# tjysdsg/speech-recognition

Hardware: AMD Instinct MI355X
Metric: frame-state loglik/s + utterances/s Viterbi decode (higher is better)
Workload: dtype f64; 1 GPU; configs[1]: 10-digit HMM, 5 states/digit, 8-mix GMM, 39-dim, 10000 utterances/GPU (999364 frames on rank 0), isolated-word decode; states=50, mixtures=8, dim=39, parallelism=utterance-sharded x1, batches_in_flight=2, process_group=single

## Files before the change

### speech-recognition_amd/csrc/gh_internal.h

```cpp
#pragma once
#include <hip/hip_runtime.h>
#include <stdint.h>
#include <stdarg.h>
#include <stdio.h>
#include <string>
#include <vector>
#include "../../include/gmmhmm.h"

void gh_set_error(const char* fmt, ...);

#define GH_HIP(call)                                                                     \
    do {                                                                                 \
        hipError_t e_ = (call);                                                          \
        if (e_ != hipSuccess) {                                                          \
            gh_set_error("%s:%d %s -> %s", __FILE__, __LINE__, #call, hipGetErrorString(e_)); \
            return (e_ == hipErrorOutOfMemory) ? GH_ERR_NOMEM : GH_ERR_HIP;              \
        }                                                                                \
    } while (0)

#define GH_REQUIRE(cond, ...)                 \
    do {                                      \
        if (!(cond)) {                        \
            gh_set_error(__VA_ARGS__);        \
            return GH_ERR_INVALID;            \
        }                                     \
    } while (0)

#define GH_LEAN_NARROW_ARCS 3

#define GH_LSE_SCALE64 184.66496523378731614
#define GH_LSE_SCALE32 1.4426950408889634074
#define GH_LSE_OFF64 (-1e300)
#define GH_LSE_OFF32 (-1e30f)
#define GH_LSE_COMPAT_BELOW64 (-745.1332191019412 * GH_LSE_SCALE64)
#define GH_LSE_BOUND_THR 0x1p-900
struct gh_lse_state { double k_mh, thr; };
__host__ __device__ inline gh_lse_state gh_lse_state_of(double mh, bool any_on, int M_pad) {
    gh_lse_state e;
    if (!any_on) { e.k_mh = 0.0; e.thr = INFINITY; return e; }
    e.k_mh = mh * GH_LSE_SCALE64;
    const double ex = (GH_LSE_COMPAT_BELOW64 - e.k_mh) * (1.0 / 128.0);
    const double t = (ex > 1000.0) ? (double)INFINITY : ((ex < -1060.0) ? 0.0 : ldexp(exp2(ex - floor(ex)), (int)floor(ex)) * (2.0 * M_pad));
    e.thr = (t > GH_LSE_BOUND_THR) ? t : GH_LSE_BOUND_THR;
    return e;
}
static inline int gh_lse_states_padded(int M_pad, int n_tiles) { return n_tiles * (16 / M_pad); }

struct gh_ctx {
    int device;
    hipStream_t stream;
    int n_cu;
    void* scratch;
    size_t scratch_bytes;
    int* d_flag;
    void* pinned;
    size_t pinned_bytes;
    double* d_fp64_tables;
    int compat;
    int last_fused = 0;
    int last_chunks;
    size_t budget_cache = 0;
    int budget_age = 0;
    void* fit_arena = nullptr;
    size_t fit_arena_bytes = 0;
    void* fit_pin = nullptr;
    void* fit_act = nullptr;
    size_t fit_act_bytes = 0;
};

int gh_scratch(gh_ctx* ctx, size_t bytes, void** out);
size_t gh_scratch_budget(gh_ctx* ctx, bool fresh = false);
int gh_pinned(gh_ctx* ctx, size_t bytes, void** out);

struct gh_gmm {
    gh_ctx* ctx;
    void* d_arena;
    int S, M, D, KP;
    std::vector<double> hA, hB, hC;
    bool host_stale = false;
    double *dA64, *dB64, *dC64;
    float *dA32, *dB32, *dC32;
    float* dCen32;
    double *dMean, *dIvar, *dLogc;
    int* dAnyPos = nullptr;
    int any_pos_host = -1;
    int M_pad, n_tiles;
    double *dApk64, *dCpk64;
    float *dApk32, *dCpk32;
    double* dCpkRel64 = nullptr;
    gh_lse_state* dLseState64 = nullptr;
    uint64_t serial = 0;
};
uint64_t gh_next_serial();

#define GH_FBCHAIN_MAX 16
struct gh_fbchain {
    int32_t n, pad;
    int32_t state[GH_FBCHAIN_MAX];
    double c0;
    double self_c[GH_FBCHAIN_MAX], next_c[GH_FBCHAIN_MAX], skip_c[GH_FBCHAIN_MAX];
};

struct gh_batch {
    gh_ctx* ctx;
    gh_dtype dtype;
    int D;
    int64_t N, U;
    void* feats;
    bool owns_feats;
    std::vector<int64_t> offsets;
    int64_t* d_offsets;
    int64_t max_T;
    bool any_T1 = false;
    void* nll;
    int nll_S;
    uint64_t nll_serial = 0;
    double* occ;
    int occ_S;
    int32_t* d_occ_states;
    double* gam;
    int gam_lanes = 0;
    bool occ_valid;
    std::vector<gh_fbchain> gam_chains;
    std::vector<int32_t> gam_utt_graph;
    std::vector<int64_t> perm;
    int64_t* d_perm;
    bool seq_seg_valid = false;
    std::vector<int32_t> seq_seg_lo, seq_seg_hi;
    std::vector<int32_t> seq_utt_K, seq_utt_word;
// ... 157 lines not shown
```

### speech-recognition_amd/csrc/gh_loglik_mfma.hip

```cpp
#include <type_traits>
#include "gh_internal.h"
#include "gh_wave.h"

namespace {

typedef double v4d __attribute__((ext_vector_type(4)));
typedef float v4f __attribute__((ext_vector_type(4)));

struct gh_loglik_blk { int64_t n0; int32_t nrows, t0, t1, pad; };

template <typename T> struct Acc;
template <> struct Acc<double> {
    typedef v4d type;
    static __device__ __forceinline__ v4d mfma(double a, double b, v4d c) {
        return __builtin_amdgcn_mfma_f64_16x16x4f64(a, b, c, 0, 0, 0);
    }
};
template <> struct Acc<float> {
    typedef v4f type;
    static __device__ __forceinline__ v4f mfma(float a, float b, v4f c) {
        return __builtin_amdgcn_mfma_f32_16x16x4f32(a, b, c, 0, 0, 0);
    }
};

struct Fp64Tables {
    double exp2[128];
    double inv[128];
    double nlog[128];
};

template <typename T> struct Dom;
template <> struct Dom<double> {
    static constexpr double inv_k = 1.0 / GH_LSE_SCALE64, off = GH_LSE_OFF64, off_test = GH_LSE_OFF64 * 0.1;
};
template <> struct Dom<float> {
    static constexpr float inv_k = (float)(1.0 / GH_LSE_SCALE32), off = GH_LSE_OFF32, off_test = GH_LSE_OFF32 * 0.1f;
};

struct LseK {
    double e3 = 2.6466421444330968834e-08;
    double l4 = -46.166241308446829036, l3 = 61.554988411262438714;
    double l2 = -92.332482616893658071, l1 = 184.66496523378731614;
    __device__ __forceinline__ void pin() {
        asm volatile("" : "+v"(e3), "+v"(l4), "+v"(l3), "+v"(l2), "+v"(l1));
    }
    __device__ __forceinline__ void pin_bnd() {
        asm volatile("" : "+v"(e3), "+v"(l4), "+s"(l3), "+s"(l2), "+s"(l1));
    }
};

__device__ __forceinline__ double logs(double s, const double* __restrict__ tab, const LseK& k) {
    const double* __restrict__ inv = tab + 128;
    const double* __restrict__ nlog = tab + 256;
    const double m = __builtin_amdgcn_frexp_mant(s);
    const int e = __builtin_amdgcn_frexp_exp(s);
    const int j = (__double2hiint(m) >> 13) & 127;
    const double rho = fma(m, inv[j], -1.0);
    double p = fma(rho, 36.932993046757463228, k.l4);
    p = fma(p, rho, k.l3);
    p = fma(p, rho, k.l2);
    p = fma(p, rho, k.l1);
    return fma(p, rho, nlog[j]) + (double)(e << 7);
}
__device__ __forceinline__ float logs(float s, const double*, const LseK&) { return __builtin_amdgcn_logf(s); }

template <int W> __device__ __forceinline__ void swap_rows(unsigned v, unsigned& a, unsigned& b) {
    if (W == 16) {
        auto r = __builtin_amdgcn_permlane16_swap(v, v, false, false);
        a = r[0]; b = r[1];
    } else {
        auto r = __builtin_amdgcn_permlane32_swap(v, v, false, false);
        a = r[0]; b = r[1];
    }
}
template <int W> __device__ __forceinline__ void pair_of(float v, float& a, float& b) {
    unsigned x, y;
    swap_rows<W>(__float_as_uint(v), x, y);
    a = __uint_as_float(x); b = __uint_as_float(y);
}
template <int W> __device__ __forceinline__ void pair_of(double v, double& a, double& b) {
    unsigned xl, yl, xh, yh;
    swap_rows<W>((unsigned)__double2loint(v), xl, yl);
    swap_rows<W>((unsigned)__double2hiint(v), xh, yh);
    a = __hiloint2double((int)xh, (int)xl); b = __hiloint2double((int)yh, (int)yl);
}
template <typename T, int W> __device__ __forceinline__ T pair_max(T v) { T a, b; pair_of<W>(v, a, b); return vmax(a, b); }
template <typename T, int W> __device__ __forceinline__ T pair_sum(T v) { T a, b; pair_of<W>(v, a, b); return a + b; }
__device__ __forceinline__ void pair_split(float v0, float v1, float& a, float& b) {
    auto r = __builtin_amdgcn_permlane16_swap(__float_as_uint(v0), __float_as_uint(v1), false, false);
    a = __uint_as_float(r[0]); b = __uint_as_float(r[1]);
}
__device__ __forceinline__ void pair_split(double v0, double v1, double& a, double& b) {
    auto lo = __builtin_amdgcn_permlane16_swap((unsigned)__double2loint(v0), (unsigned)__double2loint(v1), false, false);
    auto hi = __builtin_amdgcn_permlane16_swap((unsigned)__double2hiint(v0), (unsigned)__double2hiint(v1), false, false);
    a = __hiloint2double((int)hi[0], (int)lo[0]); b = __hiloint2double((int)hi[1], (int)lo[1]);
}
template <typename T> __device__ __forceinline__ T pair_sum_split(T v0, T v1) { T a, b; pair_split(v0, v1, a, b); return a + b; }
template <typename T> __device__ __forceinline__ T pair_max_split(T v0, T v1) { T a, b; pair_split(v0, v1, a, b); return vmax(a, b); }

template <typename T> __device__ __forceinline__ T nll_of(T mx, T sm, const double* tab, T inf_below, const LseK& k) {
    const T v = (mx + logs(sm, tab, k)) * -Dom<T>::inv_k;
    return (mx < inf_below) ? T(INFINITY) : v;
}

template <typename T, typename V> __device__ __forceinline__ T lane_max(const V& a) { return vmax(vmax(a[0], a[1]), vmax(a[2], a[3])); }
template <typename T, typename V> __device__ __forceinline__ T lane_terms(const V& a, T m, const double* tab, const LseK& k) {
    return (exp2s(a[0] - m, tab, k.e3) + exp2s(a[1] - m, tab, k.e3)) + (exp2s(a[2] - m, tab, k.e3) + exp2s(a[3] - m, tab, k.e3));
}
template <typename T, typename V>
__device__ __forceinline__ void tile_lse(const V& a, int width, T& mx, T& sm, const double* tab, const LseK& k) {
    T m = lane_max<T, V>(a);
    if (width >= 2) m = pair_max<T, 16>(m);
    if (width >= 4) m = pair_max<T, 32>(m);
    T e = lane_terms<T, V>(a, m, tab, k);
    if (width >= 2) e = pair_sum<T, 16>(e);
    if (width >= 4) e = pair_sum<T, 32>(e);
    mx = m;
    sm = e;
}

template <typename T, typename V, int W>
__device__ __forceinline__ void wide_lse(const V& acc0, const V& acc1, T& mxs, T& sm, const double* tab, const LseK& k) {
    mxs = pair_max_split(lane_max<T, V>(acc0), lane_max<T, V>(acc1));
    if (W >= 4) mxs = pair_max<T, 32>(mxs);
    T mx0, mx1;
    pair_of<16>(mxs, mx0, mx1);
    sm = pair_sum_split(lane_terms<T, V>(acc0, mx0, tab, k), lane_terms<T, V>(acc1, mx1, tab, k));
    if (W >= 4) sm = pair_sum<T, 32>(sm);
}

template <typename T, typename V> __device__ __forceinline__ T lane_terms0(const V& a, const double* tab, const LseK& k) {
    return (exp2s(a[0], tab, k.e3) + exp2s(a[1], tab, k.e3)) + (exp2s(a[2], tab, k.e3) + exp2s(a[3], tab, k.e3));
}
template <typename T> __device__ __forceinline__ T nll_bnd(T k_mh, T sm, const double* tab, const LseK& k) {
    return (k_mh + logs(sm, tab, k)) * -Dom<T>::inv_k;
}
template <typename T> __device__ __forceinline__ T nll_cold(T mx, T sm, T k_mh, const double* tab, T inf_below, const LseK& k) {
    const T v = ((mx + logs(sm, tab, k)) + k_mh) * -Dom<T>::inv_k;
    return (mx + k_mh < inf_below) ? T(INFINITY) : v;
}
__device__ __forceinline__ bool wave_any(bool p) { return __builtin_amdgcn_ballot_w64(p) != 0; }
__device__ __forceinline__ void cold_block() { asm volatile("; log-sum-exp redo (max-shifted)" ::: "memory"); }

__device__ __forceinline__ float exp2s_fe(double y) { return __builtin_amdgcn_exp2f((float)y * 0.0078125f); }
template <int W> __device__ __forceinline__ float pair_sum_f(float v) { float a, b; pair_of<W>(v, a, b); return a + b; }
// ... 136 lines not shown
            *((!CHK || s < S) ? orow0 + s : dummy) = nll_of_fe(mx, sm, inf_below);
            tile_lse_fe<V>(acc1, 1, mx, sm);
            *((!CHK || s < S) ? orow1 + s : dummy) = nll_of_fe(mx, sm, inf_below);
        }
    } else if (FE && MP <= 16) {
        if constexpr (FE) {
            constexpr int width = MP / 4;
            double mx0, mx1; float sm0, sm1;
            tile_lse_fe<V>(acc0, width, mx0, sm0);
            tile_lse_fe<V>(acc1, width, mx1, sm1);
            const bool odd = q & 1;
            const int s = (16 / MP) * t + q / width;
            const double v = nll_of_fe(odd ? mx1 : mx0, odd ? sm1 : sm0, inf_below);
            *(((q & (width - 1)) < 2 && (!CHK || s < S)) ? (odd ? orow1 : orow0) + s : dummy) = v;
        }
    } else if (FE) {
        if constexpr (FE) {
            const bool last = (t + 1) % tiles_per_state == 0;
            const int s = t / tiles_per_state;
#pragma unroll
            for (int c = 0; c < 2; ++c) {
                double mx; float smf;
                tile_lse_fe<V>(c ? acc1 : acc0, 4, mx, smf);
                const double d = run_mx[c] - mx;
                const float e = exp2s_fe((d > 0.0) ? -d : d);
                const float rs = (float)run_sm[c];
                run_sm[c] = (double)((d > 0.0) ? fmaf(smf, e, rs) : fmaf(rs, e, smf));
                run_mx[c] = (d > 0.0) ? run_mx[c] : mx;
            }
            const bool odd = q & 1;
            const double v = nll_of_fe(odd ? run_mx[1] : run_mx[0], (float)(odd ? run_sm[1] : run_sm[0]), inf_below);
            *((last && q < 2) ? (odd ? orow1 : orow0) + s : dummy) = v;
#pragma unroll
            for (int c = 0; c < 2; ++c) {
                run_mx[c] = last ? Dom<T>::off : run_mx[c];
                run_sm[c] = last ? T(0) : run_sm[c];
            }
        }
    } else if (MP == 4) {
        T mx, sm;
        const int s = 4 * t + q;
        tile_lse<T, V>(acc0, 1, mx, sm, tab, k);
        *((!CHK || s < S) ? orow0 + s : dummy) = nll_of<T>(mx, sm, tab, inf_below, k);
        tile_lse<T, V>(acc1, 1, mx, sm, tab, k);
        *((!CHK || s < S) ? orow1 + s : dummy) = nll_of<T>(mx, sm, tab, inf_below, k);
    } else if (MP <= 16) {
        constexpr int width = MP / 4;
        T mxs, sm;
        wide_lse<T, V, width>(acc0, acc1, mxs, sm, tab, k);
        const bool odd = q & 1;
        const int s = (16 / MP) * t + q / width;
        const T v = nll_of<T>(mxs, sm, tab, inf_below, k);
        *(((q & (width - 1)) < 2 && (!CHK || s < S)) ? (odd ? orow1 : orow0) + s : dummy) = v;
    } else {
        const bool last = (t + 1) % tiles_per_state == 0;
        const int s = t / tiles_per_state;
#pragma unroll
        for (int c = 0; c < 2; ++c) {
            T mx, sm;
            tile_lse<T, V>(c ? acc1 : acc0, 4, mx, sm, tab, k);
            const T d = run_mx[c] - mx;
            const T e = exp2s((d > T(0)) ? -d : d, tab, k.e3);
            run_sm[c] = (d > T(0)) ? fma(sm, e, run_sm[c]) : fma(run_sm[c], e, sm);
            run_mx[c] = (d > T(0)) ? run_mx[c] : mx;
        }
        const bool odd = q & 1;
        const T v = nll_of<T>(odd ? run_mx[1] : run_mx[0], odd ? run_sm[1] : run_sm[0], tab, inf_below, k);
        *((last && q < 2) ? (odd ? orow1 : orow0) + s : dummy) = v;
#pragma unroll
        for (int c = 0; c < 2; ++c) {
            run_mx[c] = last ? Dom<T>::off : run_mx[c];
            run_sm[c] = last ? T(0) : run_sm[c];
        }
    }
}

#ifndef GH_MF_SGB
#define GH_MF_SGB 0
#endif
#ifndef GH_MF_KSTEP
#define GH_MF_KSTEP 1
#endif
#define GH_MF_KSTEP_MASK (0x002 | 0x004 | 0x040 | 0x080 | 0x100 | 0x200 | 0x400)
template <typename T, int KS, int MP, bool MULTI, bool FE = false, bool BND = false>
__global__ __launch_bounds__(64, (sizeof(T) == 4 ? 3 : 1)) void loglik_mfma_kernel(const T* __restrict__ X, int64_t N, int D,
                                                         const T* __restrict__ Apk, const T* __restrict__ Cpk,
                                                         int n_tiles, int S, int M_pad, int chunk_tiles,
                                                         const double* __restrict__ tables, int tab_off,
                                                         T* __restrict__ out, int bpw,
                                                         const gh_loglik_blk* __restrict__ blk_tab, int64_t n_blk,
                                                         const T* __restrict__ cen, T inf_below,
                                                         const gh_lse_state* __restrict__ st_glob, int st_off) {
    static_assert(!BND || (sizeof(T) == 8 && !FE && MP >= 2 && MP <= 16), "the pack-time bound is for the default fp64 log-sum-exp, one tile per state");
    typedef typename Acc<T>::type V;
#ifndef GH_MF_RING32
#define GH_MF_RING32 2
#endif
#ifndef GH_MF_RING64
#define GH_MF_RING64 1
#endif
    constexpr int R = KS / (sizeof(T) == 4 ? GH_MF_RING32 : GH_MF_RING64);
    constexpr bool KSTEP = GH_MF_KSTEP >= 2 || (GH_MF_KSTEP == 1 && BND);
    extern __shared__ __attribute__((aligned(16))) unsigned char smem_raw[];
    T* lds = reinterpret_cast<T*>(smem_raw);
    const int lane = threadIdx.x;
    const int f = lane & 15, q = lane >> 4;
    const int64_t n_blocks = (N + 31) / 32;
    int64_t n0 = (int64_t)blockIdx.x * (MULTI ? bpw : 1) * 32;
#ifdef GH_MF_TIMING
    long long tk[5], tw[2];
    tk[0] = clock64(); tw[0] = wall_clock64();
#endif
    int nrows = 0;
    const bool subset = MULTI && blk_tab != nullptr;
    const int64_t kb0 = (int64_t)blockIdx.x * (MULTI ? bpw : 1);
    int t_lo = subset ? blk_tab[kb0].t0 : 0, t_hi = n_tiles, nxt_t0 = 0;
    double* tab = reinterpret_cast<double*>(smem_raw + tab_off);
    double* st_tab = reinterpret_cast<double*>(smem_raw + st_off);
    const int tiles_per_state = (MP <= 16) ? 1 : M_pad / 16;
    const int SC = (MP <= 16) ? chunk_tiles * (16 / (MP <= 16 ? MP : 16)) : chunk_tiles / tiles_per_state;
    const int st_n = n_tiles * (16 / (MP <= 16 ? MP : 16));
    int st_s0 = -1;
    auto stage_states = [&](int s0) {
        if constexpr (BND) {
            const int cnt = (st_n - s0 < SC) ? st_n - s0 : SC;
            const bool compat = inf_below > Dom<T>::off_test;
            gh_lse_state e[2];
#pragma unroll
            for (int it = 0; it < 2; ++it) e[it] = (lane + 64 * it < cnt) ? st_glob[s0 + lane + 64 * it] : gh_lse_state{0.0, 0.0};
#pragma unroll
            for (int it = 0; it < 2; ++it)
                if (lane + 64 * it < cnt) {
                    st_tab[2 * (lane + 64 * it)] = e[it].k_mh;
                    st_tab[2 * (lane + 64 * it) + 1] = compat ? e[it].thr : ((e[it].thr == 0.0) ? 0.0 : GH_LSE_BOUND_THR);
                }
            st_s0 = s0;
        }
    };
    auto states_landed = [&]() { if constexpr (BND) __builtin_amdgcn_s_waitcnt(0x0F70); };
    if (BND) stage_states(t_lo * (16 / (MP <= 16 ? MP : 16)));
    if (sizeof(T) == 8 && MP != 1) {
        double tr[6];
#pragma unroll
        for (int it = 0; it < 6; ++it) tr[it] = tables[lane + 64 * it];
#pragma unroll
        for (int it = 0; it < 6; ++it) tab[lane + 64 * it] = tr[it];
    }
    auto stage_frames = [&]() {
        const int nelem = nrows * D;
        const T* src = X + n0 * D;
        T xr[KS];
#pragma unroll
        for (int it = 0; it < KS; ++it) {
            const int i = lane + 64 * it;
            xr[it] = (i < nelem) ? src[i] : T(0);
        }
#pragma unroll
        for (int it = 0; it < KS; ++it) {
            const int i = lane + 64 * it;
            if (i < nelem) lds[i] = xr[it];
        }
        __syncthreads();
    };
    constexpr int KQ = KS / 2;
    T b[2][KS];
    T cen_r[KQ];
#pragma unroll
    for (int j = 0; j < KQ; ++j) cen_r[j] = (sizeof(T) == 4 && cen) ? cen[4 * j + q] : T(0);
    auto build_b = [&]() {
#pragma unroll
        for (int c = 0; c < 2; ++c) {
            const int row = 16 * c + f;
#pragma unroll
            for (int j = 0; j < KQ; ++j) {
                const int d = 4 * j + q;
                T v = (row < nrows && d < D) ? lds[row * D + d] : T(0);
                if (sizeof(T) == 4) v = (row < nrows && d < D) ? v - cen_r[j] : T(0);
                b[c][j] = v * v;
                b[c][KQ + j] = v;
            }
        }
        __syncthreads();
    };

    const int RS = (S <= SC) ? S : SC;
    T* dummy = lds + 32 * RS + lane;
    T run_mx[2] = {Dom<T>::off, Dom<T>::off}, run_sm[2] = {T(0), T(0)};
    LseK lse_k;
    if (sizeof(T) == 8 && !MULTI && !FE && MP != 1) { if (BND) lse_k.pin_bnd(); else lse_k.pin(); }
    int chunk_s0 = 0;
    int subset_cnt = 0;

    T ring[R];
#pragma unroll
    for (int j = 0; j < R; ++j) ring[j] = Apk[((int64_t)t_lo * KS + j) * 64 + lane];
    V c_a, c_b, p0, p1;
#pragma unroll
    for (int r = 0; r < 4; ++r) c_a[r] = Cpk[t_lo * 16 + 4 * q + r];

    auto mfma_tile = [&](int t, V& acc0, V& acc1, const V& c_use, V& c_load) {
        const int tn = (!MULTI || t + 1 < t_hi) ? t + 1 : nxt_t0;
        const global_ptr<T> cp = uniform_ptr(Cpk + (unsigned)(tn * 16));
#pragma unroll
        for (int r = 0; r < 4; ++r) c_load[r] = cp[4 * q + r];
        constexpr int WIN = 4096 / (64 * (int)sizeof(T)), NW = (KS + WIN - 1) / WIN;
        global_ptr<T> a_cur[NW], a_nxt[NW];
#pragma unroll
        for (int w = 0; w < NW; ++w) {
            a_cur[w] = uniform_ptr(Apk + (unsigned)(t * (KS * 64) + w * (WIN * 64)));
            a_nxt[w] = uniform_ptr(Apk + (unsigned)(tn * (KS * 64) + w * (WIN * 64)));
        }
#pragma unroll
        for (int ks = 0; ks < KS; ++ks) {
            const T a = ring[ks % R];
#ifdef GH_MF_NOMFMA
            if (ks == 0) { acc0 = c_use; acc1 = c_use; }
            if (ks % 8 == 0) { acc0[ks % 4] += a * b[0][ks]; acc1[ks % 4] += a * b[1][ks]; }
            else asm volatile("" :: "v"(a));
#else
            acc0 = Acc<T>::mfma(a, b[0][ks], ks == 0 ? c_use : acc0);
            acc1 = Acc<T>::mfma(a, b[1][ks], ks == 0 ? c_use : acc1);
#endif
#ifndef GH_MF_NOLOAD
            ring[ks % R] = (ks + R < KS) ? a_cur[(ks + R) / WIN][((ks + R) % WIN) * 64 + lane]
                                         : a_nxt[(ks + R - KS) / WIN][((ks + R - KS) % WIN) * 64 + lane];
#endif
            if constexpr (KSTEP) __builtin_amdgcn_sched_barrier(GH_MF_KSTEP_MASK);
        }
    };
    auto flush = [&]() {
        const int cnt = subset ? subset_cnt : ((chunk_s0 + SC < S) ? chunk_s0 + SC : S) - chunk_s0;
        __syncthreads();
        if (cnt == S && !subset) {
            typedef T V16 __attribute__((ext_vector_type(16 / sizeof(T))));
            constexpr int VE = 16 / sizeof(T);
            T* dst = out + n0 * S;
            const int total = nrows * S;
            const int nvec = total / VE;
#pragma unroll 4
            for (int i = lane; i < nvec; i += 64)
                reinterpret_cast<V16*>(dst)[i] = reinterpret_cast<const V16*>(lds)[i];
            for (int i = nvec * VE + lane; i < total; i += 64) dst[i] = lds[i];
        } else if (cnt > 0) {
            const int total = nrows * cnt;
            for (int i = lane; i < total; i += 64) {
                const int r = i / cnt, j = i - r * cnt;
                out[(n0 + r) * S + chunk_s0 + j] = lds[r * RS + j];
            }
        }
        __syncthreads();
        chunk_s0 += SC;
    };

    const int nb = MULTI ? bpw : 1;
    int64_t staged_n0 = -1;
    for (int ib = 0; ib < nb; ++ib, n0 += 32) {
        if (subset) {
            const int64_t k = kb0 + ib;
            if (k >= n_blk) break;
            const gh_loglik_blk bd = blk_tab[k];
            n0 = bd.n0; nrows = bd.nrows; t_lo = bd.t0; t_hi = bd.t1;
            nxt_t0 = (ib + 1 < nb && k + 1 < n_blk) ? blk_tab[k + 1].t0 : bd.t0;
        } else {
            if (MULTI && n0 >= N) break;
            nrows = (int)((N - n0 < 32) ? (N - n0) : 32);
        }
        if (!(subset && ib > 0 && n0 == staged_n0)) {
#ifdef GH_MF_PRIO
            __builtin_amdgcn_s_setprio(3);
#endif
            stage_frames();
            build_b();
#ifdef GH_MF_PRIO
            __builtin_amdgcn_s_setprio(0);
#endif
            staged_n0 = n0;
        }
        chunk_s0 = (MP <= 16) ? t_lo * (16 / (MP <= 16 ? MP : 16)) : t_lo / tiles_per_state;
        if (subset) {
            const int s_end = (MP <= 16) ? t_hi * (16 / (MP <= 16 ? MP : 16)) : t_hi / tiles_per_state;
            subset_cnt = ((s_end < S) ? s_end : S) - chunk_s0;
        }
        if (BND && st_s0 != chunk_s0) { stage_states(chunk_s0); states_landed(); __syncthreads(); }
#ifdef GH_MF_TIMING
        tk[1] = clock64();
        tk[2] = tk[1];
#endif
        auto epi = [&](const V& e0, const V& e1, int t, auto chk) {
            tile_epilogue<T, V, MP, FE, decltype(chk)::value, BND>(e0, e1, t, f, q, S, RS, chunk_s0, tiles_per_state, lds, dummy, tab, run_mx, run_sm, inf_below, lse_k, st_tab);
#pragma unroll
            for (int i = 0; i < (GH_MF_SGB ? 2 * KS : 0); ++i) {
                __builtin_amdgcn_sched_group_barrier(0x008, 1, 0);
                __builtin_amdgcn_sched_group_barrier(0x002, sizeof(T) == 8 ? 5 : 3, 0);
            }
            if (!subset && (t + 1) % chunk_tiles == 0 && t + 1 < n_tiles) {
                flush();
                if (BND) { stage_states(chunk_s0); states_landed(); __syncthreads(); }
            }
        };
        V r0, r1;
        const int tb = MULTI ? t_lo : 0, te = MULTI ? t_hi : n_tiles;
        mfma_tile(tb, p0, p1, c_a, c_b);
        if (sizeof(T) == 8) {
            int t = tb + 1;
            for (; t + 1 < te; t += 2) {
                mfma_tile(t, r0, r1, c_b, c_a);
                epi(p0, p1, t - 1, std::false_type());
                mfma_tile(t + 1, p0, p1, c_a, c_b);
                epi(r0, r1, t, std::false_type());
            }
            if (t < te) {
                mfma_tile(t, r0, r1, c_b, c_a);
                epi(p0, p1, t - 1, std::false_type());
                epi(r0, r1, t, std::true_type());
            } else {
                epi(p0, p1, te - 1, std::true_type());
                if (MULTI) c_a = c_b;
            }
        } else {
            for (int t = tb + 1; t < te; ++t) {
                mfma_tile(t, r0, r1, c_b, c_a);
                epi(p0, p1, t - 1, std::false_type());
                p0 = r0;
                p1 = r1;
                c_b = c_a;
            }
            epi(p0, p1, te - 1, std::true_type());
            if (MULTI) c_a = c_b;
        }
#ifdef GH_MF_TIMING
        tk[3] = clock64();
#endif
        flush();
#ifdef GH_MF_TIMING
        tk[4] = clock64(); tw[1] = wall_clock64();
        if (lane == 0 && S >= 8) {
            T* o = out + n0 * S;
            for (int i = 0; i < 5; ++i) o[i] = (T)(double)(tk[i] - tk[0]);
            o[5] = (T)(double)(tw[0] & 0xffffffffffll); o[6] = (T)(double)(tw[1] - tw[0]);
            o[7] = (T)(double)__builtin_amdgcn_s_getreg((4 << 0) | (0 << 6) | (31 << 11));
        }
#endif
    }
}

static void chunk_shape(const gh_gmm* g, int* chunk_tiles_out, int* SC_out) {
    const int M_pad = g->M_pad, n_tiles = g->n_tiles, S = g->S;
    int chunk_tiles;
    if (M_pad <= 16) {
        const int spt = 16 / M_pad;
        chunk_tiles = (S <= 64) ? n_tiles : std::max(1, 64 / spt);
    } else {
        const int tps = M_pad / 16;
        chunk_tiles = (S <= 64) ? n_tiles : 64 * tps;
    }
    *chunk_tiles_out = chunk_tiles;
    *SC_out = (M_pad <= 16) ? chunk_tiles * (16 / M_pad) : chunk_tiles / (M_pad / 16);
}

static int build_blk_table(const gh_gmm* g, const gh_batch* b, int SC, const int32_t* st_lo, const int32_t* st_hi,
                           const int64_t* rng_off, std::vector<gh_loglik_blk>& tabv, int* max_tiles_out,
                           const uint8_t* include = nullptr) {
    const int M_pad = g->M_pad, S = g->S;
    int max_tiles = 1;
    std::vector<std::pair<int, int>> runs;
    for (int64_t u = 0; u < b->U; ++u) {
        if (include && !include[u]) continue;
        runs.clear();
        const int64_t r0 = rng_off ? rng_off[u] : u, r1 = rng_off ? rng_off[u + 1] : u + 1;
        for (int64_t r = r0; r < r1; ++r) {
            const int lo = st_lo[r], hi = st_hi[r];
            if (lo < 0 || hi > S || lo >= hi) { gh_set_error("gh_loglik_subset: utterance %lld has state range [%d, %d)", (long long)u, lo, hi); return GH_ERR_INVALID; }
            int t0, t1;
            if (M_pad <= 16) { const int spt = 16 / M_pad; t0 = lo / spt; t1 = (hi + spt - 1) / spt; }
            else { const int tps = M_pad / 16; t0 = lo * tps; t1 = hi * tps; }
            runs.push_back({t0, t1});
        }
        std::sort(runs.begin(), runs.end());
        size_t w = 0;
        for (size_t i = 0; i < runs.size(); ++i) {
            if (w > 0 && runs[i].first <= runs[w - 1].second) runs[w - 1].second = std::max(runs[w - 1].second, runs[i].second);
            else runs[w++] = runs[i];
        }
        runs.resize(w);
        for (const auto& tr : runs) {
            const int t0 = tr.first, t1 = tr.second;
            const int span = (M_pad <= 16) ? (t1 - t0) * (16 / M_pad) : (t1 - t0) / (M_pad / 16);
            if (span > SC) return 1;
            max_tiles = std::max(max_tiles, t1 - t0);
        }
        for (int64_t f = b->offsets[u]; f < b->offsets[u + 1]; f += 32)
            for (const auto& tr : runs)
                tabv.push_back(gh_loglik_blk{f, (int32_t)std::min<int64_t>(32, b->offsets[u + 1] - f), tr.first, tr.second, 0});
    }
    *max_tiles_out = max_tiles;
    return GH_OK;
}

static bool lse_bound_enabled() {
    const char* e = getenv("GMMHMM_LSE_BOUND");
    return !(e && e[0] == '0' && e[1] == 0);
}

template <typename T>
int launch_mfma_t(gh_ctx* ctx, const gh_gmm* g, gh_batch* b, const T* Apk, const T* Cpk, const T* CpkRel, const int32_t* st_lo,
                  const int32_t* st_hi, const T* cen, const int64_t* rng_off, const gh_loglik_plan* plan) {
    const int64_t N = b->N;
    if (N == 0) return GH_OK;
    const int KS = g->KP / 2;
    const int M_pad = g->M_pad, n_tiles = g->n_tiles, S = g->S;
    int chunk_tiles, SC;
    chunk_shape(g, &chunk_tiles, &SC);
    size_t lds = ((size_t)32 * std::max(std::min(SC, S), g->D) + 64) * sizeof(T);
    lds = (lds + 15) & ~size_t(15);
    const int tab_off = (int)lds;
    if (sizeof(T) == 8 && M_pad != 1) lds += 384 * sizeof(double);
    const bool bnd = sizeof(T) == 8 && M_pad != 1 && M_pad <= 16 && !((ctx->compat & 2) && M_pad >= 4) && CpkRel && g->dLseState64 && lse_bound_enabled();
    const int st_off = (int)lds;
    if (bnd) lds += (size_t)std::min(SC, gh_lse_states_padded(M_pad, n_tiles)) * sizeof(gh_lse_state);
    const double* tables = ctx->d_fp64_tables;
    const T inf_below = (ctx->compat & 1) ? (T)(-745.1332191019412 * (sizeof(T) == 8 ? GH_LSE_SCALE64 : GH_LSE_SCALE32)) : Dom<T>::off_test;
    gh_loglik_blk* d_blk = nullptr;
    int64_t n_blk = 0;
    int max_tiles = n_tiles;
    if (plan) {
        d_blk = static_cast<gh_loglik_blk*>(plan->d_blk);
        n_blk = plan->n_blk;
        max_tiles = plan->max_tiles;
        if (n_blk == 0) return GH_OK;
    } else if (st_lo) {
        std::vector<gh_loglik_blk> tabv;
        int rc = build_blk_table(g, b, SC, st_lo, st_hi, rng_off, tabv, &max_tiles);
        if (rc) return rc;
        n_blk = (int64_t)tabv.size();
        if (n_blk == 0) return GH_OK;
        void* base;
        rc = gh_scratch(ctx, tabv.size() * sizeof(gh_loglik_blk), &base);
        if (rc) return rc;
        d_blk = static_cast<gh_loglik_blk*>(base);
        GH_HIP(hipMemcpyAsync(d_blk, tabv.data(), tabv.size() * sizeof(gh_loglik_blk), hipMemcpyHostToDevice, ctx->stream));
        GH_HIP(hipStreamSynchronize(ctx->stream));
    }
    const bool subset = plan || st_lo;
    const int64_t n_blocks = subset ? n_blk : (N + 31) / 32;
    const int per_block = std::max(1, max_tiles * KS * 2);
    int bpw = (int)std::max<int64_t>(1, std::min<int64_t>(8, (512 + per_block - 1) / per_block));
    if (const char* e = getenv("GMMHMM_LOGLIK_BPW")) bpw = std::max(1, std::min(16, atoi(e)));
    if (subset) bpw = std::max(bpw, 2);
    const unsigned grid = (unsigned)((n_blocks + bpw - 1) / bpw);
    const T* X = static_cast<const T*>(b->feats);
    T* out = static_cast<T*>(b->nll);
    const bool fe = sizeof(T) == 8 && (ctx->compat & 2) && M_pad >= 4;
#define GH_MF_LAUNCH1(ks, mp, multi, fe_, bnd_)                                                                          \
    hipLaunchKernelGGL((loglik_mfma_kernel<T, ks, mp, multi, fe_, bnd_>), dim3(grid), dim3(64), lds, ctx->stream, X, N, g->D, \
                       Apk, bnd ? CpkRel : Cpk, n_tiles, S, M_pad, chunk_tiles, tables, tab_off, out, bpw, d_blk, n_blk, cen, \
                       inf_below, g->dLseState64, st_off)
#define GH_MF_LAUNCH(ks, mp)                                                                                             \
    do {                                                                                                                 \
        constexpr bool f64 = sizeof(T) == 8;                                                                             \
        if (fe && f64 && mp >= 4) {                                                                                      \
            if (bpw > 1) GH_MF_LAUNCH1(ks, mp, true, (f64 && mp >= 4), false);                                           \
            else GH_MF_LAUNCH1(ks, mp, false, (f64 && mp >= 4), false);                                                  \
        } else if (bnd && f64 && mp != 1 && mp <= 16) {                                                                  \
            if (bpw > 1) GH_MF_LAUNCH1(ks, mp, true, false, (f64 && mp != 1 && mp <= 16));                               \
            else GH_MF_LAUNCH1(ks, mp, false, false, (f64 && mp != 1 && mp <= 16));                                      \
        } else if (bpw > 1)                                                                                              \
            GH_MF_LAUNCH1(ks, mp, true, false, false);                                                                   \
        else                                                                                                             \
            GH_MF_LAUNCH1(ks, mp, false, false, false);                                                                  \
    } while (0)
#define GH_MF_CASE(ks)                                   \
    case ks:                                             \
        switch (M_pad) {                                 \
            case 1: GH_MF_LAUNCH(ks, 1); break;          \
            case 2: GH_MF_LAUNCH(ks, 2); break;          \
            case 4: GH_MF_LAUNCH(ks, 4); break;          \
            case 8: GH_MF_LAUNCH(ks, 8); break;          \
            case 16: GH_MF_LAUNCH(ks, 16); break;        \
            default: GH_MF_LAUNCH(ks, 32); break;        \
        }                                                \
        break;
    switch (KS) {
        GH_MF_CASE(2)
        GH_MF_CASE(4)
        GH_MF_CASE(8)
        GH_MF_CASE(12)
        GH_MF_CASE(20)
        GH_MF_CASE(24)
        GH_MF_CASE(32)
        default:
            return 1;
    }
#undef GH_MF_CASE
#undef GH_MF_LAUNCH
#undef GH_MF_LAUNCH1
    GH_HIP(hipGetLastError());
    return GH_OK;
}

}

int gh_launch_loglik_mfma(gh_ctx* ctx, const gh_gmm* g, gh_batch* b, const int32_t* st_lo, const int32_t* st_hi,
                          const int64_t* rng_off, const gh_loglik_plan* plan) {
    if (!g->dApk64) return 1;
    b->nll_serial = g->serial;
    if (b->dtype == GH_F64) return launch_mfma_t<double>(ctx, g, b, g->dApk64, g->dCpk64, g->dCpkRel64, st_lo, st_hi, nullptr, rng_off, plan);
    return launch_mfma_t<float>(ctx, g, b, g->dApk32, g->dCpk32, (const float*)nullptr, st_lo, st_hi, g->dCen32, rng_off, plan);
}

int gh_loglik_plan_build(gh_ctx* ctx, const gh_gmm* g, const gh_batch* b, const int32_t* st_lo, const int32_t* st_hi,
                         const int64_t* rng_off, gh_loglik_plan* out, const uint8_t* include) {
    out->d_blk = nullptr; out->n_blk = 0; out->max_tiles = 1;
    if (!g->dApk64) return 1;
    const int KS = g->KP / 2;
    if (KS != 2 && KS != 4 && KS != 8 && KS != 12 && KS != 20 && KS != 24 && KS != 32) return 1;
    int chunk_tiles, SC;
    chunk_shape(g, &chunk_tiles, &SC);
    std::vector<gh_loglik_blk> tabv;
    int rc = build_blk_table(g, b, SC, st_lo, st_hi, rng_off, tabv, &out->max_tiles, include);
    if (rc) return rc;
    out->n_blk = (int64_t)tabv.size();
    if (tabv.empty()) return GH_OK;
    GH_HIP(hipMalloc(&out->d_blk, tabv.size() * sizeof(gh_loglik_blk)));
    GH_HIP(hipMemcpy(out->d_blk, tabv.data(), tabv.size() * sizeof(gh_loglik_blk), hipMemcpyHostToDevice));
    return GH_OK;
}

void gh_loglik_plan_free(gh_loglik_plan* p) {
    if (p && p->d_blk) hipFree(p->d_blk);
    if (p) { p->d_blk = nullptr; p->n_blk = 0; }
}
```

### speech-recognition_amd/csrc/gh_model.hip

```cpp
#include "gh_internal.h"
#include <atomic>
#include "gh_host.h"

uint64_t gh_next_serial() {
    static std::atomic<uint64_t> counter{0};
    return ++counter;
}

__host__ __device__ inline void gh_pack_lse_state(const double* c, const double* logc, int M, int M_pad, double* rel, gh_lse_state* st) {
    double mh = -INFINITY;
    bool any_on = false, all_nan = (M == M_pad);
    for (int m = 0; m < M; ++m) {
        if (c[m] - c[m] == 0.0 && logc[m] - logc[m] == 0.0 && c[m] * GH_LSE_SCALE64 > GH_LSE_OFF64) { any_on = true; mh = (logc[m] > mh) ? logc[m] : mh; }
        all_nan = all_nan && c[m] != c[m];
    }
    *st = gh_lse_state_of(mh, any_on, M_pad);
    for (int m = 0; m < M; ++m) {
        const double r = (c[m] - mh) * GH_LSE_SCALE64;
        if (!any_on) rel[m] = all_nan ? c[m] : GH_LSE_OFF64;
        else rel[m] = (c[m] == -INFINITY) ? GH_LSE_OFF64 : ((r > GH_LSE_OFF64) ? r : GH_LSE_OFF64) + (c[m] != c[m] ? c[m] : 0.0);
    }
}

extern "C" int gh_gmm_create(gh_ctx* ctx, int S, int M, int D, const double* mean, const double* var,
// ... 7 lines not shown
    for (const int kp : {4, 8, 16, 24, 40, 48, 64})
        if (KP <= kp) { KP = kp; break; }
    gh_gmm* g = new gh_gmm();
    g->ctx = ctx;
    g->d_arena = nullptr;
    g->S = S; g->M = M; g->D = D; g->KP = KP;
    g->hA.assign((size_t)G * KP, 0.0);
    g->hB.assign((size_t)G * KP, 0.0);
    g->hC.assign(G, 0.0);
    std::vector<double> ivar((size_t)G * D), logc(G);
    const double log2pi = std::log(2.0 * M_PI);
    for (int i = 0; i < G; ++i) {
        double sum_logv = 0, sum_m2 = 0;
        for (int d = 0; d < D; ++d) {
            const double v = var[(size_t)i * D + d], mu = mean[(size_t)i * D + d];
            if (v == 0) {
                delete g;
                gh_set_error("gh_gmm_create: var[%d,%d,%d]=%g (singular covariance)",
                             i / M, i % M, d, v);
                return GH_ERR_INVALID;
            }
            const double iv = 1.0 / v;
            ivar[(size_t)i * D + d] = iv;
            g->hA[(size_t)i * KP + d] = -0.5 * iv;
            g->hB[(size_t)i * KP + d] = mu * iv;
            sum_logv += std::log(v);
            sum_m2 += mu * mu * iv;
        }
        logc[i] = std::log(weight[i]) - 0.5 * (D * log2pi + sum_logv);
        g->hC[i] = logc[i] - 0.5 * sum_m2;
    }
    std::vector<float> cen32(KP, 0.f);
    for (int d = 0; d < D; ++d) {
        long double acc = 0;
        int cnt = 0;
        for (int i = 0; i < G; ++i) {
            const double mu = mean[(size_t)i * D + d];
            if (std::isfinite(mu)) { acc += mu; ++cnt; }
        }
        cen32[d] = cnt ? (float)(double)(acc / cnt) : 0.f;
        if (!std::isfinite(cen32[d])) cen32[d] = 0.f;
    }
    std::vector<double> hB32((size_t)G * KP, 0.0), hC32(G, 0.0);
    for (int i = 0; i < G; ++i) {
        double sum_m2 = 0;
        for (int d = 0; d < D; ++d) {
            const double iv = ivar[(size_t)i * D + d], mu = mean[(size_t)i * D + d] - (double)cen32[d];
            hB32[(size_t)i * KP + d] = mu * iv;
            sum_m2 += mu * mu * iv;
        }
        hC32[i] = logc[i] - 0.5 * sum_m2;
    }
    std::vector<float> fA(g->hA.begin(), g->hA.end()), fB(hB32.begin(), hB32.end()), fC(hC32.begin(), hC32.end());
    int M_pad = 1;
    if (M <= 16) { while (M_pad < M) M_pad <<= 1; } else { M_pad = (M + 15) & ~15; }
    const int n_tiles = (S * M_pad + 15) / 16, KS = KP / 2;
    g->M_pad = M_pad;
    g->n_tiles = n_tiles;
    g->dApk64 = nullptr; g->dCpk64 = nullptr; g->dApk32 = nullptr; g->dCpk32 = nullptr; g->dCen32 = nullptr;
    std::vector<double> apk64((size_t)(n_tiles + 2) * KS * 64, 0.0), cpk64((size_t)(n_tiles + 2) * 16, GH_LSE_OFF64);
    std::vector<float> apk32(apk64.size(), 0.f), cpk32(cpk64.size(), GH_LSE_OFF32);
    for (int t = 0; t < n_tiles; ++t)
        for (int j = 0; j < 16; ++j) {
            const int gp = t * 16 + j, s = gp / M_pad, m = gp % M_pad;
            if (s >= S || m >= M) continue;
            const int go = s * M + m;
            const double c = g->hC[go], c32 = hC32[go];
            cpk64[gp] = (c == -INFINITY) ? GH_LSE_OFF64 : std::max(c * GH_LSE_SCALE64, GH_LSE_OFF64);
            cpk32[gp] = (c32 == -INFINITY) ? GH_LSE_OFF32 : (float)std::max(c32 * GH_LSE_SCALE32, (double)GH_LSE_OFF32);
            const int row64 = (j >> 2) + 4 * (j & 3), row32 = j;
            for (int ks = 0; ks < KS; ++ks)
                for (int kq = 0; kq < 4; ++kq) {
                    const int kk = 4 * ks + kq;
                    const double v = kk < KP ? g->hA[(size_t)go * KP + kk] : g->hB[(size_t)go * KP + kk - KP];
                    const double v32 = kk < KP ? v : hB32[(size_t)go * KP + kk - KP];
                    apk64[((size_t)t * KS + ks) * 64 + kq * 16 + row64] = v * GH_LSE_SCALE64;
                    apk32[((size_t)t * KS + ks) * 64 + kq * 16 + row32] = (float)(v32 * GH_LSE_SCALE32);
                }
        }
    const bool lse_bound = M_pad >= 2 && M_pad <= 16;
    std::vector<double> cpkrel64(lse_bound ? cpk64.size() : 0, GH_LSE_OFF64);
    std::vector<gh_lse_state> lse_state(lse_bound ? gh_lse_states_padded(M_pad, n_tiles) : 0, gh_lse_state{0.0, 0.0});
    for (int s = 0; lse_bound && s < S; ++s) gh_pack_lse_state(&g->hC[(size_t)s * M], &logc[(size_t)s * M], M, M_pad, &cpkrel64[(size_t)s * M_pad], &lse_state[s]);
    std::vector<double> vmean(mean, mean + (size_t)G * D);
    std::vector<int> anypos(1, 0);
    for (int i = 0; i < G; ++i) if (logc[i] > 0) anypos[0] = 1;
    UploadArena ar;
    ar.add(&g->dA64, g->hA); ar.add(&g->dB64, g->hB); ar.add(&g->dC64, g->hC);
    ar.add(&g->dA32, fA); ar.add(&g->dB32, fB); ar.add(&g->dC32, fC); ar.add(&g->dCen32, cen32);
    ar.add(&g->dMean, vmean); ar.add(&g->dIvar, ivar); ar.add(&g->dLogc, logc); ar.add(&g->dAnyPos, anypos);
    g->any_pos_host = anypos[0];
    ar.add(&g->dApk64, apk64); ar.add(&g->dCpk64, cpk64); ar.add(&g->dApk32, apk32); ar.add(&g->dCpk32, cpk32);
    ar.add(&g->dCpkRel64, cpkrel64); ar.add(&g->dLseState64, lse_state);
    const int rc = ar.commit(&g->d_arena);
    if (rc) {
        gh_gmm_destroy(g);
        return rc;
    }
    g->serial = gh_next_serial();
    *out = g;
    return GH_OK;
}

__global__ __launch_bounds__(1024) void gmm_centre_kernel(const double* __restrict__ mean, int G, int D, int KP, float* __restrict__ cen32,
                                                          int* __restrict__ any_pos) {
    __shared__ double s_acc[16];
    __shared__ int s_cnt[16];
    const int d = blockIdx.x, tid = threadIdx.x, lane = tid & 63, wave = tid >> 6;
    if (d == 0 && tid == 0) *any_pos = 0;
    double acc = 0;
    int cnt = 0;
    if (d < D)
        for (int i = tid; i < G; i += 1024) {
            const double mu = mean[(size_t)i * D + d];
            if (mu - mu == 0.0) { acc += mu; ++cnt; }
        }
#pragma unroll
    for (int o = 32; o >= 1; o >>= 1) { acc += __shfl_xor(acc, o); cnt += __shfl_xor(cnt, o); }
    if (lane == 0) { s_acc[wave] = acc; s_cnt[wave] = cnt; }
    __syncthreads();
    if (tid == 0) {
        double a = 0;
        int n = 0;
        for (int w = 0; w < 16; ++w) { a += s_acc[w]; n += s_cnt[w]; }
        float c = n ? (float)(a / n) : 0.f;
        if (!(c - c == 0.f)) c = 0.f;
        cen32[d] = c;
    }
}

struct gmm_dev_view {
    int* any_pos;
    int S, M, D, KP, M_pad, n_tiles;
    double *A64, *B64, *C64, *Mean, *Ivar, *Logc, *Apk64, *Cpk64, *CpkRel64;
    gh_lse_state* LseState64;
    float *A32, *B32, *C32, *Apk32, *Cpk32;
    const float* cen32;
};

__global__ void gmm_pack_plain_kernel(gmm_dev_view v, const double* __restrict__ mean, const double* __restrict__ var,
                                      const double* __restrict__ weight, int* __restrict__ flag) {
    const int i = blockIdx.x * blockDim.x + threadIdx.x;
    const int G = v.S * v.M;
    if (i >= G) return;
    const int D = v.D, KP = v.KP;
    const double log2pi = 1.8378770664093454836;
    double sum_logv = 0, sum_m2 = 0, sum_m2c = 0;
    for (int d = 0; d < D; ++d) {
        const double vv = var[(size_t)i * D + d], mu = mean[(size_t)i * D + d];
        if (vv == 0) atomicOr(flag, 16);
        const double iv = 1.0 / vv;
        const double muc = mu - (double)v.cen32[d];
        v.Mean[(size_t)i * D + d] = mu;
        v.Ivar[(size_t)i * D + d] = iv;
        v.A64[(size_t)i * KP + d] = -0.5 * iv;
        v.B64[(size_t)i * KP + d] = mu * iv;
        v.A32[(size_t)i * KP + d] = (float)(-0.5 * iv);
        v.B32[(size_t)i * KP + d] = (float)(muc * iv);
        sum_logv += log(vv);
        sum_m2 += mu * mu * iv;
        sum_m2c += muc * muc * iv;
    }
    const double logc = log(weight[i]) - 0.5 * (D * log2pi + sum_logv);
    v.Logc[i] = logc;
    if (logc > 0) atomicOr(v.any_pos, 1);
    const double c = logc - 0.5 * sum_m2, c32 = logc - 0.5 * sum_m2c;
    v.C64[i] = c;
    v.C32[i] = (float)c32;
    const int s = i / v.M, m = i - s * v.M;
    const int gp = s * v.M_pad + m;
    v.Cpk64[gp] = (c == -INFINITY) ? GH_LSE_OFF64 : fmax(c * GH_LSE_SCALE64, GH_LSE_OFF64) + (c != c ? c : 0.0);
    v.Cpk32[gp] = (c32 == -INFINITY) ? GH_LSE_OFF32 : (float)(fmax(c32 * GH_LSE_SCALE32, (double)GH_LSE_OFF32) + (c32 != c32 ? c32 : 0.0));
}

__global__ void gmm_pack_lse_kernel(gmm_dev_view v) {
    const int s = blockIdx.x * blockDim.x + threadIdx.x;
    if (s >= v.S) return;
    gh_pack_lse_state(v.C64 + (size_t)s * v.M, v.Logc + (size_t)s * v.M, v.M, v.M_pad, v.CpkRel64 + (size_t)s * v.M_pad, v.LseState64 + s);
}

__global__ void gmm_pack_operands_kernel(gmm_dev_view v) {
    const int64_t idx = (int64_t)blockIdx.x * blockDim.x + threadIdx.x;
    const int K2 = 2 * v.KP;
    const int64_t total = (int64_t)v.n_tiles * 16 * K2;
    if (idx >= total) return;
    const int gp = (int)(idx / K2), kk = (int)(idx - (int64_t)gp * K2);
    const int s = gp / v.M_pad, m = gp - s * v.M_pad;
    if (s >= v.S || m >= v.M) return;
    const int go = s * v.M + m;
    const int t = gp >> 4, j = gp & 15;
    const int KS = v.KP / 2, ks = kk >> 2, kq = kk & 3;
    const int row64 = (j >> 2) + 4 * (j & 3), row32 = j;
    const double a64 = kk < v.KP ? v.A64[(size_t)go * v.KP + kk] : v.B64[(size_t)go * v.KP + kk - v.KP];
    double a32 = a64;
    if (kk >= v.KP) {
        const int d = kk - v.KP;
        a32 = d < v.D ? (v.Mean[(size_t)go * v.D + d] - (double)v.cen32[d]) * v.Ivar[(size_t)go * v.D + d] : 0.0;
    }
    v.Apk64[((size_t)t * KS + ks) * 64 + kq * 16 + row64] = a64 * GH_LSE_SCALE64;
    v.Apk32[((size_t)t * KS + ks) * 64 + kq * 16 + row32] = (float)(a32 * GH_LSE_SCALE32);
}

int gh_gmm_update_dev(gh_ctx* ctx, gh_gmm* g, const double* d_mean, const double* d_var, const double* d_weight, int* d_flag) {
    const int G = g->S * g->M;
    hipStream_t st = ctx->stream;
    gmm_dev_view v;
    v.S = g->S; v.M = g->M; v.D = g->D; v.KP = g->KP; v.M_pad = g->M_pad; v.n_tiles = g->n_tiles;
    v.A64 = g->dA64; v.B64 = g->dB64; v.C64 = g->dC64; v.Mean = g->dMean; v.Ivar = g->dIvar; v.Logc = g->dLogc;
    v.Apk64 = g->dApk64; v.Cpk64 = g->dCpk64; v.A32 = g->dA32; v.B32 = g->dB32; v.C32 = g->dC32;
    v.Apk32 = g->dApk32; v.Cpk32 = g->dCpk32; v.cen32 = g->dCen32; v.any_pos = g->dAnyPos;
    v.CpkRel64 = g->dCpkRel64; v.LseState64 = g->dLseState64;
    g->any_pos_host = -1;
    hipLaunchKernelGGL(gmm_centre_kernel, dim3(g->KP), dim3(1024), 0, st, d_mean, G, g->D, g->KP, g->dCen32, g->dAnyPos);
    hipLaunchKernelGGL(gmm_pack_plain_kernel, dim3((G + 63) / 64), dim3(64), 0, st, v, d_mean, d_var, d_weight, d_flag);
    if (g->dCpkRel64) hipLaunchKernelGGL(gmm_pack_lse_kernel, dim3((g->S + 63) / 64), dim3(64), 0, st, v);
    const int64_t total = (int64_t)g->n_tiles * 16 * 2 * g->KP;
    hipLaunchKernelGGL(gmm_pack_operands_kernel, dim3((unsigned)((total + 255) / 256)), dim3(256), 0, st, v);
    GH_HIP(hipGetLastError());
    g->host_stale = true;
    g->serial = gh_next_serial();
    return GH_OK;
}

extern "C" int gh_gmm_update(gh_ctx* ctx, gh_gmm* g, const double* mean, const double* var, const double* weight) {
    GH_REQUIRE(ctx && g && mean && var && weight, "gh_gmm_update: NULL argument");
    GH_HIP(hipSetDevice(ctx->device));
    const size_t G = (size_t)g->S * g->M, nd = G * g->D;
    for (size_t i = 0; i < nd; ++i)
        GH_REQUIRE(var[i] != 0, "gh_gmm_update: var[%zu,%zu,%zu]=0 (singular covariance)", i / g->D / g->M, i / g->D % g->M, i % g->D);
    void* base;
    int rc = gh_scratch(ctx, (2 * nd + G) * 8, &base);
    if (rc) return rc;
    double* d = static_cast<double*>(base);
    GH_HIP(hipMemcpyAsync(d, mean, nd * 8, hipMemcpyHostToDevice, ctx->stream));
    GH_HIP(hipMemcpyAsync(d + nd, var, nd * 8, hipMemcpyHostToDevice, ctx->stream));
    GH_HIP(hipMemcpyAsync(d + 2 * nd, weight, G * 8, hipMemcpyHostToDevice, ctx->stream));
    rc = gh_gmm_update_dev(ctx, g, d, d + nd, d + 2 * nd, ctx->d_flag);
    if (rc) return rc;
    GH_HIP(hipStreamSynchronize(ctx->stream));
    return GH_OK;
}

extern "C" void gh_gmm_destroy(gh_gmm* g) {
    if (!g) return;
    hipSetDevice(g->ctx->device);
    hipFree(g->d_arena);
    delete g;
}

static int batch_common(gh_ctx* ctx, gh_dtype dtype, int D, int64_t N, int64_t U, const int64_t* off,
                        gh_batch** out) {
    GH_REQUIRE(ctx && out && off, "gh_batch: NULL argument");
    GH_REQUIRE(dtype == GH_F32 || dtype == GH_F64, "gh_batch: bad dtype %d", (int)dtype);
    GH_REQUIRE(D > 0 && N >= 0 && U >= 0, "gh_batch: D=%d N=%lld U=%lld", D, (long long)N, (long long)U);
    GH_REQUIRE(off[0] == 0 && off[U] == N, "gh_batch: utt_offsets must run from 0 to N");
    for (int64_t u = 0; u < U; ++u)
        GH_REQUIRE(off[u + 1] >= off[u], "gh_batch: utt_offsets not monotone at %lld", (long long)u);
    GH_HIP(hipSetDevice(ctx->device));
    gh_batch* b = new gh_batch();
    b->ctx = ctx; b->dtype = dtype; b->D = D; b->N = N; b->U = U;
    b->feats = nullptr; b->owns_feats = false; b->nll = nullptr; b->nll_S = 0; b->d_offsets = nullptr;
    b->occ = nullptr;
    b->occ_S = 0;
    b->gam = nullptr;
    b->occ_valid = false;
    b->d_occ_states = nullptr;
    b->offsets.assign(off, off + U + 1);
    b->max_T = 0;
    for (int64_t u = 0; u < U; ++u) {
        b->max_T = std::max(b->max_T, off[u + 1] - off[u]);
        if (off[u + 1] - off[u] == 1) b->any_T1 = true;
    }
    b->perm.resize(U);
    std::iota(b->perm.begin(), b->perm.end(), (int64_t)0);
    std::stable_sort(b->perm.begin(), b->perm.end(), [&](int64_t x, int64_t y) {
        return off[x + 1] - off[x] > off[y + 1] - off[y];
    });
    b->d_perm = nullptr;
    int rc = upload(&b->d_offsets, b->offsets);
    if (!rc) rc = upload(&b->d_perm, b->perm);
    if (rc) { delete b; return rc; }
    *out = b;
    return GH_OK;
// ... 403 lines not shown
```

Measured before the change: 44.13 billion frame-state loglik/s.

## Fold per-mixture constant into a padded K slot of the MFMA operand

Uses the unused padded feature dimension (KP > D, here 39 padded to 40) to carry the per-Gaussian constant term in the packed A operand. The B operand gets a matching 1 in that slot, so the MFMA accumulates the constant directly. This removes the per-tile Cpk loads and the accumulator initialisation from them. A second slot carries the LSE k_mh shift for the bound path. The log helper is also rewritten to fold the exponent add into an fma. The change adds template variants and packing logic on both the host and device update paths, and it risks precision or layout mismatches in those slots.

```diff
diff --git a/speech-recognition_amd/csrc/gh_internal.h b/speech-recognition_amd/csrc/gh_internal.h
--- a/speech-recognition_amd/csrc/gh_internal.h
+++ b/speech-recognition_amd/csrc/gh_internal.h
@@ -45,6 +45,7 @@
     return e;
 }
 static inline int gh_lse_states_padded(int M_pad, int n_tiles) { return n_tiles * (16 / M_pad); }
+__host__ __device__ inline double gh_cslot64(double cpk, bool has_rel, double rel) { return has_rel ? rel : cpk; }
 
 struct gh_ctx {
     int device;
diff --git a/speech-recognition_amd/csrc/gh_loglik_mfma.hip b/speech-recognition_amd/csrc/gh_loglik_mfma.hip
--- a/speech-recognition_amd/csrc/gh_loglik_mfma.hip
+++ b/speech-recognition_amd/csrc/gh_loglik_mfma.hip
@@ -60,7 +60,7 @@
     p = fma(p, rho, k.l3);
     p = fma(p, rho, k.l2);
     p = fma(p, rho, k.l1);
-    return fma(p, rho, nlog[j]) + (double)(e << 7);
+    return fma((double)e, 128.0, fma(p, rho, nlog[j]));
 }
 __device__ __forceinline__ float logs(float s, const double*, const LseK&) { return __builtin_amdgcn_logf(s); }
 
@@ -363,7 +363,7 @@
 #define GH_MF_KSTEP 1
 #endif
 #define GH_MF_KSTEP_MASK (0x002 | 0x004 | 0x040 | 0x080 | 0x100 | 0x200 | 0x400)
-template <typename T, int KS, int MP, bool MULTI, bool FE = false, bool BND = false>
+template <typename T, int KS, int MP, bool MULTI, bool FE = false, bool BND = false, bool CS = false>
 __global__ __launch_bounds__(64, (sizeof(T) == 4 ? 3 : 1)) void loglik_mfma_kernel(const T* __restrict__ X, int64_t N, int D,
                                                          const T* __restrict__ Apk, const T* __restrict__ Cpk,
                                                          int n_tiles, int S, int M_pad, int chunk_tiles,
@@ -460,6 +460,11 @@
                 b[c][j] = v * v;
                 b[c][KQ + j] = v;
             }
+            if constexpr (CS) {
+                const T one = (row < nrows) ? T(1) : T(0);
+                b[c][KS - 1] = (q == 3) ? one : b[c][KS - 1];
+                if (sizeof(T) == 8 && !BND && MP >= 2 && MP <= 16) b[c][KQ - 1] = (q == 3) ? one : b[c][KQ - 1];
+            }
         }
         __syncthreads();
     };
@@ -476,14 +481,19 @@
 #pragma unroll
     for (int j = 0; j < R; ++j) ring[j] = Apk[((int64_t)t_lo * KS + j) * 64 + lane];
     V c_a, c_b, p0, p1;
-#pragma unroll
-    for (int r = 0; r < 4; ++r) c_a[r] = Cpk[t_lo * 16 + 4 * q + r];
+    if constexpr (!CS) {
+#pragma unroll
+        for (int r = 0; r < 4; ++r) c_a[r] = Cpk[t_lo * 16 + 4 * q + r];
+    }
 
     auto mfma_tile = [&](int t, V& acc0, V& acc1, const V& c_use, V& c_load) {
         const int tn = (!MULTI || t + 1 < t_hi) ? t + 1 : nxt_t0;
-        const global_ptr<T> cp = uniform_ptr(Cpk + (unsigned)(tn * 16));
-#pragma unroll
-        for (int r = 0; r < 4; ++r) c_load[r] = cp[4 * q + r];
+        if constexpr (!CS) {
+            const global_ptr<T> cp = uniform_ptr(Cpk + (unsigned)(tn * 16));
+#pragma unroll
+            for (int r = 0; r < 4; ++r) c_load[r] = cp[4 * q + r];
+        }
+        const V zero = {T(0), T(0), T(0), T(0)};
         constexpr int WIN = 4096 / (64 * (int)sizeof(T)), NW = (KS + WIN - 1) / WIN;
         global_ptr<T> a_cur[NW], a_nxt[NW];
 #pragma unroll
@@ -495,12 +505,12 @@
         for (int ks = 0; ks < KS; ++ks) {
             const T a = ring[ks % R];
 #ifdef GH_MF_NOMFMA
-            if (ks == 0) { acc0 = c_use; acc1 = c_use; }
+            if (ks == 0) { acc0 = CS ? zero : c_use; acc1 = CS ? zero : c_use; }
             if (ks % 8 == 0) { acc0[ks % 4] += a * b[0][ks]; acc1[ks % 4] += a * b[1][ks]; }
             else asm volatile("" :: "v"(a));
 #else
-            acc0 = Acc<T>::mfma(a, b[0][ks], ks == 0 ? c_use : acc0);
-            acc1 = Acc<T>::mfma(a, b[1][ks], ks == 0 ? c_use : acc1);
+            acc0 = Acc<T>::mfma(a, b[0][ks], ks == 0 ? (CS ? zero : c_use) : acc0);
+            acc1 = Acc<T>::mfma(a, b[1][ks], ks == 0 ? (CS ? zero : c_use) : acc1);
 #endif
 #ifndef GH_MF_NOLOAD
             ring[ks % R] = (ks + R < KS) ? a_cur[(ks + R) / WIN][((ks + R) % WIN) * 64 + lane]
@@ -596,7 +606,7 @@
                 epi(r0, r1, t, std::true_type());
             } else {
                 epi(p0, p1, te - 1, std::true_type());
-                if (MULTI) c_a = c_b;
+                if (MULTI && !CS) c_a = c_b;
             }
         } else {
             for (int t = tb + 1; t < te; ++t) {
@@ -604,10 +614,10 @@
                 epi(p0, p1, t - 1, std::false_type());
                 p0 = r0;
                 p1 = r1;
-                c_b = c_a;
+                if (!CS) c_b = c_a;
             }
             epi(p0, p1, te - 1, std::true_type());
-            if (MULTI) c_a = c_b;
+            if (MULTI && !CS) c_a = c_b;
         }
 #ifdef GH_MF_TIMING
         tk[3] = clock64();
@@ -682,6 +692,10 @@
     const char* e = getenv("GMMHMM_LSE_BOUND");
     return !(e && e[0] == '0' && e[1] == 0);
 }
+static bool cslot_enabled() {
+    const char* e = getenv("GMMHMM_LOGLIK_CSLOT");
+    return !(e && e[0] == '0' && e[1] == 0);
+}
 
 template <typename T>
 int launch_mfma_t(gh_ctx* ctx, const gh_gmm* g, gh_batch* b, const T* Apk, const T* Cpk, const T* CpkRel, const int32_t* st_lo,
@@ -697,6 +711,7 @@
     const int tab_off = (int)lds;
     if (sizeof(T) == 8 && M_pad != 1) lds += 384 * sizeof(double);
     const bool bnd = sizeof(T) == 8 && M_pad != 1 && M_pad <= 16 && !((ctx->compat & 2) && M_pad >= 4) && CpkRel && g->dLseState64 && lse_bound_enabled();
+    const bool cslot = g->KP > g->D && cslot_enabled();
     const int st_off = (int)lds;
     if (bnd) lds += (size_t)std::min(SC, gh_lse_states_padded(M_pad, n_tiles)) * sizeof(gh_lse_state);
     const double* tables = ctx->d_fp64_tables;
@@ -732,10 +747,23 @@
     const T* X = static_cast<const T*>(b->feats);
     T* out = static_cast<T*>(b->nll);
     const bool fe = sizeof(T) == 8 && (ctx->compat & 2) && M_pad >= 4;
-#define GH_MF_LAUNCH1(ks, mp, multi, fe_, bnd_)                                                                          \
-    hipLaunchKernelGGL((loglik_mfma_kernel<T, ks, mp, multi, fe_, bnd_>), dim3(grid), dim3(64), lds, ctx->stream, X, N, g->D, \
+#define GH_MF_LAUNCH2(ks, mp, multi, fe_, bnd_, cs_)                                                                     \
+    hipLaunchKernelGGL((loglik_mfma_kernel<T, ks, mp, multi, fe_, bnd_, cs_>), dim3(grid), dim3(64), lds, ctx->stream, X, N, g->D, \
                        Apk, bnd ? CpkRel : Cpk, n_tiles, S, M_pad, chunk_tiles, tables, tab_off, out, bpw, d_blk, n_blk, cen, \
                        inf_below, g->dLseState64, st_off)
+#define GH_MF_LAUNCH1(ks, mp, multi, fe_, bnd_)                                                                          \
+    do {                                                                                                                 \
+              \
+              \
+               \
+              \
+        constexpr bool cs_kept = !(sizeof(T) == 8 && ks == 8 && mp == 2) && mp != 32;                                    \
+        if constexpr (cs_kept) {                                                                                         \
+            if (cslot) GH_MF_LAUNCH2(ks, mp, multi, fe_, bnd_, true);                                                    \
+            else GH_MF_LAUNCH2(ks, mp, multi, fe_, bnd_, false);                                                         \
+        } else                                                                                                           \
+            GH_MF_LAUNCH2(ks, mp, multi, fe_, bnd_, false);                                                              \
+    } while (0)
 #define GH_MF_LAUNCH(ks, mp)                                                                                             \
     do {                                                                                                                 \
         constexpr bool f64 = sizeof(T) == 8;                                                                             \
@@ -775,6 +803,7 @@
 #undef GH_MF_CASE
 #undef GH_MF_LAUNCH
 #undef GH_MF_LAUNCH1
+#undef GH_MF_LAUNCH2
     GH_HIP(hipGetLastError());
     return GH_OK;
 }
diff --git a/speech-recognition_amd/csrc/gh_model.hip b/speech-recognition_amd/csrc/gh_model.hip
--- a/speech-recognition_amd/csrc/gh_model.hip
+++ b/speech-recognition_amd/csrc/gh_model.hip
@@ -113,6 +113,14 @@
     std::vector<double> cpkrel64(lse_bound ? cpk64.size() : 0, GH_LSE_OFF64);
     std::vector<gh_lse_state> lse_state(lse_bound ? gh_lse_states_padded(M_pad, n_tiles) : 0, gh_lse_state{0.0, 0.0});
     for (int s = 0; lse_bound && s < S; ++s) gh_pack_lse_state(&g->hC[(size_t)s * M], &logc[(size_t)s * M], M, M_pad, &cpkrel64[(size_t)s * M_pad], &lse_state[s]);
+    if (KP > D)
+        for (int gp = 0; gp < n_tiles * 16; ++gp) {
+            const int t = gp >> 4, j = gp & 15, row64 = (j >> 2) + 4 * (j & 3), row32 = j;
+            const size_t sq = ((size_t)t * KS + KS / 2 - 1) * 64 + 48, lin = ((size_t)t * KS + KS - 1) * 64 + 48;
+            apk64[lin + row64] = gh_cslot64(cpk64[gp], lse_bound, lse_bound ? cpkrel64[gp] : 0.0);
+            if (lse_bound) apk64[sq + row64] = lse_state[gp / M_pad].k_mh;
+            apk32[lin + row32] = cpk32[gp];
+        }
     std::vector<double> vmean(mean, mean + (size_t)G * D);
     std::vector<int> anypos(1, 0);
     for (int i = 0; i < G; ++i) if (logc[i] > 0) anypos[0] = 1;
@@ -228,8 +236,17 @@
         const int d = kk - v.KP;
         a32 = d < v.D ? (v.Mean[(size_t)go * v.D + d] - (double)v.cen32[d]) * v.Ivar[(size_t)go * v.D + d] : 0.0;
     }
-    v.Apk64[((size_t)t * KS + ks) * 64 + kq * 16 + row64] = a64 * GH_LSE_SCALE64;
-    v.Apk32[((size_t)t * KS + ks) * 64 + kq * 16 + row32] = (float)(a32 * GH_LSE_SCALE32);
+    double p64 = a64 * GH_LSE_SCALE64;
+    float p32 = (float)(a32 * GH_LSE_SCALE32);
+    if (v.KP > v.D && kk == K2 - 1) {
+        p64 = gh_cslot64(v.Cpk64[gp], v.CpkRel64 != nullptr, v.CpkRel64 ? v.CpkRel64[gp] : 0.0);
+        p32 = v.Cpk32[gp];
+    } else if (v.KP > v.D && kk == v.KP - 1) {
+        p64 = v.LseState64 ? v.LseState64[s].k_mh : 0.0;
+        p32 = 0.f;
+    }
+    v.Apk64[((size_t)t * KS + ks) * 64 + kq * 16 + row64] = p64;
+    v.Apk32[((size_t)t * KS + ks) * 64 + kq * 16 + row32] = p32;
 }
 
 int gh_gmm_update_dev(gh_ctx* ctx, gh_gmm* g, const double* d_mean, const double* d_var, const double* d_weight, int* d_flag) {
```

Result: no change. 44.39 billion frame-state loglik/s (median of 6 runs) (+0.6%).
